# XJTU-Power-AI/charginghub-env

Measured on AMD Instinct MI355X. Metric: env-steps/sec at 65 536 parallel envs, higher is better.
Workload: dtype f64; 1 GPU; 65536 envs x hub [20 fast, 25 slow] (BASELINE.json configs[3]), fcev_permeate 0.01, random policy resident in HBM, reset every 96 steps, Philox streams; envs_per_gpu=65536, obs_dim=13, act_dim=47, work_order=XCD-aware (tiles, tail and level workgroups in contiguous eighths per XCD), graph=on, collective=none

## Files before the change

### charginghub-env_amd/csrc/chub_kernels.hip

```cpp
#include <hip/hip_runtime.h>
#include <hip/hip_ext.h>
#include <stdint.h>

#include "chub_device.h"
#include "chub_plan.h"

namespace chub {

typedef uint32_t u32x4 __attribute__((ext_vector_type(4)));
typedef uint32_t u32x2 __attribute__((ext_vector_type(2)));

__device__ __forceinline__ bool in_group(const StepArgs &sa, int64_t env) { return !sa.env_mask || sa.env_mask[env] != 0; }
__device__ __forceinline__ uint32_t env_clk(const StepArgs &sa, int64_t n_envs, int64_t env) {
    return sa.env_clk[(int64_t) (sa.tick & 1u) * n_envs + env];
}
__device__ __forceinline__ int64_t range_len(const StepArgs &sa) { return (int64_t) sa.env_hi - sa.env_lo + 1; }
__device__ __forceinline__ bool range_unit(const StepArgs &sa, int64_t i, int segments, int &seg, int64_t &env) {
    const int64_t R = range_len(sa);
    if (i >= (int64_t) segments * R) return false;
    seg = (i >= R ? 1 : 0) + (i >= 2 * R ? 1 : 0);
    env = sa.env_lo + (i - (int64_t) seg * R);
    return true;
}

// ... 1192 lines not shown
        float r_min, r_chg, r_max;
        if (MODE == MODE_COMPAT) {
            SumsF32 r = {0.0f, 0.0f, 0.0f};
            r.add(s_a, s_b, s_c, S);
            r_min = r.mn; r_chg = r.chg; r_max = r.mx;
        } else {
            SumsI64 r = {0, 0, 0};
            r.add(s_u, s_v, s_w, S);
            r_min = fixed64_to_kw(r.mn); r_chg = fixed64_to_kw(r.chg); r_max = fixed64_to_kw(r.mx);
        }
        rec_store(st.rec, sidx, r_min, r_chg, r_max, pkd_make(s_hdr[2], s_hdr[1], cars));
    }
}

template <bool RESET, int MODE>
__global__ __launch_bounds__(256) void k_slot_unit_any(const DevCtx *__restrict__ ctx, StepArgs sa, int k) {
    typedef float f32x2 __attribute__((ext_vector_type(2)));
    const HubParams &hp = ctx->hp;
    const SlotArrays &sl = ctx->sl;
    const StationArrays &st = ctx->st;
    const Tables &tb = ctx->tb;
    __shared__ float s_a[256], s_b[256], s_c[256];
    __shared__ uint32_t s_u[256], s_v[256], s_w[256];
    __shared__ float s_soc[256];
    __shared__ uint64_t s_ball[8];
    __shared__ int s_hdr[4];
    __shared__ int s_cnt;
    __shared__ float s_em[kMaxPiles], s_pw[kMaxPiles];
    __shared__ uint16_t s_cb[kMaxPiles], s_rk[kMaxPiles];
    const int tid = threadIdx.x, lane = tid & 63, wave = tid >> 6;
    const int env = (int) blockIdx.x;
    const int64_t N = hp.n_envs;
    if (!in_group(sa, env)) return;
    const int S = hp.S[k], chunks = (S + 255) >> 8;
    const bool fast = hp.type[k] == 0, cp = hp.constant_charging != 0;
    const int hub0 = k ? hp.S[0] : 0;
    const uint32_t idx0 = MODE == MODE_PHILOX ? (uint32_t) env * (uint32_t) (hp.S[0] + hp.S[1]) + (uint32_t) hub0
                                              : (uint32_t) hp.base[k] + (uint32_t) env * (uint32_t) S;
    const uint32_t sidx = (uint32_t) k * (uint32_t) N + (uint32_t) env;
    CHUB_G(const float) cls = tb.cls[k];
    if (tid == 0) s_cnt = 0;
    __syncthreads();

    float load = 0.0f;
    if (!RESET && sa.load_mode) {
        for (int slot = tid; slot < S; slot += 256) {
            const uint32_t idx = idx0 + (uint32_t) slot;
            float t_target = 0.0f, t_soc = 0.0f;
            int tl;
            if (MODE == MODE_COMPAT) {
                const u32x4 hot = ((CHUB_G(u32x4)) sl.hot)[idx];
                t_soc = __uint_as_float(hot.z);
                tl = hot_tl(hot.w);
                if (tl > 0) t_target = tb.ttab[k][hot_level(hot.w)];
            } else {
                const uint32_t w0 = sl.hot[idx];
                tl = ps_tl(w0);
                if (tl > 0) {
                    t_soc = (*(CHUB_G(const f32x2)) ((CHUB_G(const char)) cls + ((size_t) ps_cls(w0) * (kClsRow * 8u) + ps_n(w0) * 8u))).y;
                    t_target = tb.ttab[k][ps_lev(w0)];
                }
            }
            s_em[slot] = tl > 0 ? emergency_of(t_target, t_soc, tl) : 0.0f;
        }
        __syncthreads();
        for (int slot = tid; slot < S; slot += 256) {
            const uint32_t idx = idx0 + (uint32_t) slot;
            float power = 0.0f;
            bool car;
            if (MODE == MODE_COMPAT) {
                const u32x4 hot = ((CHUB_G(u32x4)) sl.hot)[idx];
                car = hot_tl(hot.w) != 0;
                power = __uint_as_float(hot.x);
            } else {
                const uint32_t w0 = sl.hot[idx];
                car = ps_tl(w0) > 0;
                if (car) power = (*(CHUB_G(const f32x2)) ((CHUB_G(const char)) cls + ((size_t) ps_cls(w0) * (kClsRow * 8u) + ps_n(w0) * 8u))).x;
            }
            const float em0 = s_em[slot];
            int rk = 0;
            for (int j = 0; j < S; j++) {
                const float ej = s_em[j];
                rk += (ej > em0 || (ej == em0 && j < slot)) ? 1 : 0;
            }
            s_rk[slot] = (uint16_t) rk;
            s_pw[rk] = car ? power : 0.0f;
            s_cb[rk] = car ? 1 : 0;
        }
        __syncthreads();
        load = catch_load(hp, sa, st, k, env, sidx);
        if (tid == 0) {
            float cum = 0.0f;
            int cars_before = 0;
            for (int q = 0; q < S; q++) {
                const int c = (int) s_cb[q];
                cum = __fadd_rn(cum, s_pw[q]);
                s_pw[q] = cum;
                s_cb[q] = (uint16_t) cars_before;
                cars_before += c;
            }
        }
        __syncthreads();
    }

    for (int c = 0; c < chunks; c++) {
        const int slot = (c << 8) + tid;
        const bool valid = slot < S;
        const uint32_t idx = idx0 + (uint32_t) slot;
        float a = 0.0f;
        if (!RESET && valid) a = sa.actions[(uint32_t) env * (uint32_t) hp.act_dim + (uint32_t) (hub0 + slot)];
        auto switched_on = [&](const float t_target, const float t_soc, const int tl) {
            if (!RESET && sa.load_mode) {
                const int rk = (int) s_rk[slot];
                return load_says_on(cp, fast, load, s_pw[rk], (int) s_cb[rk]);
            }
            return a >= kActOnThreshold || must_charge(t_target, t_soc, tl);
        };
        bool car;
        if constexpr (MODE == MODE_COMPAT) {
            CompatSlot s = {};
            float t_target = 0.0f;
            if (!RESET && valid) {
                const u32x4 hot = ((CHUB_G(u32x4)) sl.hot)[idx];
                s = CompatSlot::unpack(hot);
                if (s.tl > 0) t_target = tb.ttab[k][hot_level(hot.w)];
            }
            const bool on = s.tl > 0 && switched_on(t_target, s.t_soc, s.tl);
            if (on) car_step_compat(s, fast, cp, hp.cc);
            remove_car_compat(s, on);
            if (RESET) s.meta = 0;
            if (valid) ((CHUB_G(u32x4)) sl.hot)[idx] = s.pack();
            car = s.tl > 0;
        } else {
            PhiloxWord s = {};
            float t_target = 0.0f, t_soc = 0.0f;
            if (!RESET && valid) {
                s.w = sl.hot[idx];
                s.tl = ps_tl(s.w);
                if (s.tl > 0) {
                    t_soc = (*(CHUB_G(const f32x2)) ((CHUB_G(const char)) cls + ((size_t) ps_cls(s.w) * (kClsRow * 8u) + ps_n(s.w) * 8u))).y;
                    t_target = tb.ttab[k][ps_lev(s.w)];
                }
            }
            const bool on = s.tl > 0 && switched_on(t_target, t_soc, s.tl);
            car_step_word(s, on);
            if (RESET) s.w = 0u;
            if (valid) sl.hot[idx] = s.w;
            car = s.tl > 0;
        }
        const uint64_t be = __ballot(valid && !car);
        if (lane == 0 && be) atomicAdd(&s_cnt, __popcll(be));
    }
    __syncthreads();
    const int empties = s_cnt;

    CompatStream rs;
    if (tid == 0) {
        Received rc;
        if (MODE == MODE_COMPAT) {
            rs.load(ctx->cr, sa.rng_cur, env);
            rc = receive_car_streams<RESET>(rs, hp, sa, tb, k, env, fast, RESET ? 0 : pkd_line(st.rec[4u * sidx + 3u]), empties);
        } else {
            rc = receive_car_word<RESET>(st.pk[sa.tick & 1u][sidx], fast, empties);
        }
        s_hdr[0] = rc.assign; s_hdr[1] = rc.flow; s_hdr[2] = rc.line;
    }
    __syncthreads();
    const int assign = s_hdr[0];

    int base = 0, cars = 0;
    SumsF32 rf = {0.0f, 0.0f, 0.0f};
    SumsI64 ri = {0, 0, 0};
    for (int c = 0; c < chunks; c++) {
        const int slot = (c << 8) + tid;
        const bool valid = slot < S;
        const uint32_t idx = idx0 + (uint32_t) slot;
        float power = 0.0f, t_target = 0.0f, t_soc = 0.0f;
        int tl = 0;
        bool charge = false;
        if (valid) {
            if (MODE == MODE_COMPAT) {
                const u32x4 hot = ((CHUB_G(u32x4)) sl.hot)[idx];
                const CompatSlot cs = CompatSlot::unpack(hot);
                power = cs.power; t_soc = cs.t_soc; tl = cs.tl; charge = cs.charge;
                if (tl > 0) t_target = tb.ttab[k][hot_level(hot.w)];
            } else {
                const uint32_t w0 = sl.hot[idx];
                tl = ps_tl(w0);
                charge = (w0 & kPsChg) != 0u;
                if (tl > 0) {
                    const f32x2 row = *(CHUB_G(const f32x2)) ((CHUB_G(const char)) cls + ((size_t) ps_cls(w0) * (kClsRow * 8u) + ps_n(w0) * 8u));
                    power = row.x; t_soc = row.y;
                    t_target = tb.ttab[k][ps_lev(w0)];
                }
            }
        }
        bool car = tl > 0;
        const bool empty = valid && !car;
        const uint64_t be = __ballot(empty);
        if (lane == 0) s_ball[wave] = be;
        __syncthreads();
        int chunk_empties = 0, rank = base + prefix_count(be);
        for (int w = 0; w < 4; w++) {
            const int n = __popcll(s_ball[w]);
            chunk_empties += n;
            rank += w < wave ? n : 0;
        }
        if (MODE == MODE_COMPAT) {
            if (tid == 0) {
                int n_new = assign - base;
                n_new = n_new < 0 ? 0 : (n_new > chunk_empties ? chunk_empties : n_new);
                for (int rr = 0; rr < n_new; rr++) {
                    const CarDraw d = draw_car_streams(rs);
                    s_soc[rr] = d.soc;
                    s_v[rr] = (uint32_t) d.lev;
                    s_w[rr] = (uint32_t) d.late;
                }
            }
            __syncthreads();
        }
        if (empty && rank < assign) {
            if (MODE == MODE_COMPAT) {
                const int r = rank - base;
                const NewCar nc = add_car_compat(fast, s_soc[r], (int) s_v[r], (int) s_w[r], cp);
                t_target = nc.t_target; t_soc = nc.t_soc; tl = nc.stay; power = nc.power;
                ((CHUB_G(u32x4)) sl.hot)[idx] = compat_slot_of(nc).pack();
            } else {
                const PhiloxCar nc = add_car_philox(hp, sa, tb, k, env, hub0 + slot);
                t_target = nc.t_target; t_soc = nc.t_soc; tl = nc.stay; power = nc.power;
                sl.hot[idx] = nc.word;
                sl.stay8[idx] = (uint8_t) nc.stay;
            }
            car = tl > 0;
        }
        const bool urgent = car && must_charge(t_target, t_soc, tl);
        const uint64_t bc = __ballot(car);
        if (lane == 0) s_ball[4 + wave] = bc;
        if (MODE == MODE_COMPAT) {
            s_a[tid] = urgent ? power : 0.0f;
            s_b[tid] = charge ? power : 0.0f;
            s_c[tid] = car ? power : 0.0f;
        } else {
            const int q = kw_to_fixed(power);
            s_u[tid] = (uint32_t) (urgent ? q : 0);
            s_v[tid] = (uint32_t) (charge ? q : 0);
            s_w[tid] = (uint32_t) (car ? q : 0);
        }
        __syncthreads();
        cars += __popcll(s_ball[4]) + __popcll(s_ball[5]) + __popcll(s_ball[6]) + __popcll(s_ball[7]);
        if (tid == 0) {
            const int n = S - (c << 8) < 256 ? S - (c << 8) : 256;
            if (MODE == MODE_COMPAT) rf.add(s_a, s_b, s_c, n);
            else ri.add(s_u, s_v, s_w, n);
        }
        base += chunk_empties;
        __syncthreads();
    }
    if (tid == 0) {
        if (MODE == MODE_COMPAT) {
            rs.store(ctx->cr, sa.rng_cur, env);
            rec_store(st.rec, sidx, rf.mn, rf.chg, rf.mx, pkd_make(s_hdr[2], s_hdr[1], cars));
        } else {
            rec_store(st.rec, sidx, fixed64_to_kw(ri.mn), fixed64_to_kw(ri.chg), fixed64_to_kw(ri.mx), pkd_make(s_hdr[2], s_hdr[1], cars));
        }
    }
}

struct PackedArgs {
    uint32_t S[2], type[2];
    uint32_t n_envs, epb, magic, cls_delta;
    CHUB_G(uint32_t) state;
    CHUB_G(uint32_t) rec;
    CHUB_G(const uint32_t) pk;
    CHUB_G(const float) actions;
    CHUB_G(const float) cls0;
    CHUB_G(const float) ttab2;
    CHUB_G(const uint32_t) car_tape;
    uint32_t key[2], gid0, tick;
    const uint32_t *tick_base;
    uint32_t late[8];
    CHUB_G(const uint8_t) env_mask;
    uint32_t blk0;
    uint32_t xcd;
    CHUB_G(float) tail_act;
    CHUB_G(uint8_t) stay8;
};

typedef const uint32_t __attribute__((address_space(4))) *chub_sptr;
__device__ __forceinline__ uint32_t sload_u32(const void *p, int i) { return ((chub_sptr) (uintptr_t) p)[i]; }
__device__ __forceinline__ bool mask_is_empty(const StepArgs &sa) { return sa.skip_count != nullptr && sload_u32(sa.skip_count, 0) == 0u; }

#ifndef CHUB_ACT_NT
#define CHUB_ACT_NT 0
#endif
#if CHUB_ACT_NT
#define CHUB_ACT_LOAD(p) __builtin_nontemporal_load(p)
#else
#define CHUB_ACT_LOAD(p) (*(p))
#endif
#ifndef CHUB_ACC_COPIES
#define CHUB_ACC_COPIES 2
#endif
constexpr int kAccCopies = CHUB_ACC_COPIES;
#ifndef CHUB_EPI_ALL
#define CHUB_EPI_ALL 1
#endif
#define CHUB_AT(T_, base, byte_off) (*(CHUB_G(T_)) ((CHUB_G(char)) (base) + (uint32_t) (byte_off)))
template <int BLOCK, int T, bool RESET, bool BIG, bool MASKED, bool FUSED, bool BITS>
__device__ __forceinline__ void packed_records(const PackedArgs &pa, const uint32_t block_local, int *s_acc, const uint32_t *s_unit, u32x4 *s_rec) {
    const int lane = threadIdx.x & 63;
    const int S0 = (int) pa.S[0], S1 = (int) pa.S[1], St = S0 + S1;
    const int epb = (int) pa.epb, N = (int) pa.n_envs;
    const int env_first = (int) block_local * epb;
    const long long *s_acc64 = (const long long *) s_acc;
    __builtin_amdgcn_fence(__ATOMIC_RELEASE, "wavefront");
    __builtin_amdgcn_wave_barrier();
    __builtin_amdgcn_fence(__ATOMIC_ACQUIRE, "wavefront");
    for (int i = lane; i < 2 * epb; i += 64) {
        const int e = i >> 1, k = i & 1;
        const int env = env_first + e;
        if (env >= N) continue;
        if (MASKED && pa.env_mask[env] == 0) continue;
        const uint32_t su = (uint32_t) (k ? N : 0) + (uint32_t) env;
        if (!RESET && !FUSED && !BITS && k == 0) {
            typedef float f32x2_ __attribute__((ext_vector_type(2)));
            const uint32_t ai = ((uint32_t) env * (uint32_t) (St + 2) + (uint32_t) St) << 2;
            const f32x2_ tv = {CHUB_AT(const float, pa.actions, ai), CHUB_AT(const float, pa.actions, ai + 4u)};
            CHUB_AT(f32x2_, pa.tail_act, (uint32_t) env << 3) = tv;
        }
        uint32_t lf = s_unit[i];
        if ((k ? S1 : S0) == 0) {
            const uint32_t pk = CHUB_AT(const uint32_t, pa.pk, su << 2);
            const bool fast = (k ? pa.type[1] : pa.type[0]) == 0;
            int want, fl;
            if (RESET) {
                fl = fast ? (int) (int16_t) (pk & 0xFFFFu) : (int) ((pk >> 16) & 0xFFFFu);
                want = fl;
            } else {
                want = dk_want(pk);
                fl = dk_flow(pk);
            }
            const int as = want < 0 ? want : 0;
            int ln = want - as;
            ln = ln < kMaxLine ? ln : kMaxLine;
            lf = pkd_make(ln, fl, 0);
        }
        u32x4 rv;
        if (!BIG) {
            int a0 = 0, a1 = 0, a2 = 0, a3 = 0;
#pragma unroll
            for (int c = 0; c < kAccCopies; c++) {
                const int *acc = s_acc + 4 * i + c * 8 * epb;
                a0 += acc[0]; a1 += acc[1]; a2 += acc[2]; a3 += acc[3];
            }
            rv = u32x4{__float_as_uint(fixed_to_kw(a0)), __float_as_uint(fixed_to_kw(a1)), __float_as_uint(fixed_to_kw(a2)),
                       lf | ((uint32_t) a3 << 16)};
        } else {
            const long long *a64 = s_acc64 + 4 * i;
            rv = u32x4{__float_as_uint((float) a64[0] * (1.0f / 524288.0f)), __float_as_uint((float) a64[1] * (1.0f / 524288.0f)),
                       __float_as_uint((float) a64[2] * (1.0f / 524288.0f)), lf | ((uint32_t) a64[3] << 16)};
        }
        CHUB_AT(u32x4, pa.rec, su << 4) = rv;
        if (FUSED) s_rec[i] = rv;
    }
}
#undef CHUB_AT

struct NoHook {
    __device__ __forceinline__ void prefetch() {}
    __device__ __forceinline__ void park() {}
};
template <int BLOCK, int T, bool TAPE, bool RESET, bool BIG, bool MASKED, bool FUSED, typename Hook, bool BITS = false, bool PIPED = false>
__device__ __forceinline__ int slot_body_packed(const HubParams &hp, const StepArgs &sa, PackedArgs &pa, const Tables &tb,
                                                const uint32_t block_local, uint32_t *q_cnt, uint32_t *q_new,
                                                uint64_t *s_ball, int *s_acc, uint32_t *s_unit, Hook &hook, u32x4 *s_rec, uint32_t *s_uinfo) {
    typedef float f32x4 __attribute__((ext_vector_type(4)));
    typedef float f32x2 __attribute__((ext_vector_type(2)));
    constexpr int WAVES = BLOCK / 64;
    const int tid = threadIdx.x;
    const int lane = tid & 63, wave = tid >> 6;
    const int S0 = (int) pa.S[0], S1 = (int) pa.S[1], St = S0 + S1;
    const int epb = (int) pa.epb, N = (int) pa.n_envs;
    const int env_first = (int) block_local * epb;
    const uint32_t idx0 = (uint32_t) env_first * (uint32_t) St;
    CHUB_STAMP_DECL(16);
    CHUB_STAMP_REAL(12);
    CHUB_STAMP(0);
#define CHUB_AT(T_, base, byte_off) (*(CHUB_G(T_)) ((CHUB_G(char)) (base) + (uint32_t) (byte_off)))

    int e_[T], k_[T], slot[T];
    bool valid[T];
    uint32_t sidx[T];
    uint32_t s2[T];
    float act[T];
    u32x2 actw[T];
    int hs_[T];
    uint32_t pk_in[T];
#pragma unroll
    for (int j = 0; j < T; j++) {
        const int v = tid + j * BLOCK;
        e_[j] = (int) (__umul24((uint32_t) v, pa.magic) >> 20);
        const int hs = v - (int) __umul24((uint32_t) e_[j], (uint32_t) St);
        k_[j] = hs >= S0 ? 1 : 0;
        hs_[j] = hs;
        slot[j] = hs - (k_[j] ? S0 : 0);
        const int env = env_first + e_[j];
        valid[j] = e_[j] < epb && env < N;
        uint32_t served = 1u;
        if (MASKED && valid[j]) served = pa.env_mask[env];
        sidx[j] = (uint32_t) (k_[j] ? N : 0) + (uint32_t) env;
        asm volatile("" : "=v"(s2[j]), "=v"(act[j]), "=v"(pk_in[j]), "=v"(actw[j]));
        if (RESET) {
            s2[j] = 0u;
            act[j] = 0.0f;
        }
        if (valid[j]) {
            if (!RESET) {
                s2[j] = CHUB_AT(uint32_t, pa.state, (idx0 + (uint32_t) v) << 2);
                if (BITS) actw[j] = CHUB_AT(const u32x2, pa.actions, ((uint32_t) env * (((uint32_t) St + 63u) >> 6) + ((uint32_t) hs >> 6)) << 3);
                else act[j] = CHUB_ACT_LOAD((CHUB_G(const float)) ((CHUB_G(const char)) pa.actions + (uint32_t) ((idx0 + (uint32_t) v + 2u * (uint32_t) env) << 2)));
            }
            pk_in[j] = CHUB_AT(const uint32_t, pa.pk, sidx[j] << 2);
        }
        if (MASKED && valid[j]) valid[j] = served != 0u;
    }
    if (!TAPE) {
        pa.tick += sload_u32(pa.tick_base, 0);
        asm volatile("" : "+s"(pa.key[0]), "+s"(pa.key[1]), "+s"(pa.gid0), "+s"(pa.tick), "+s"(pa.late[0]), "+s"(pa.late[1]), "+s"(pa.late[2]),
                          "+s"(pa.late[3]), "+s"(pa.late[4]), "+s"(pa.late[5]), "+s"(pa.late[6]), "+s"(pa.late[7]));
    }
    CHUB_STAMP(1);
    if (FUSED) hook.prefetch();
    if (tid == 0) q_cnt[0] = 0;
    for (int i = tid; i < (BIG ? 16 : 8 * kAccCopies) * epb; i += BLOCK) s_acc[i] = 0;
    long long *s_acc64 = (long long *) s_acc;

    uint32_t w0[T];
    int tl[T];
    bool stays[T];
    f32x4 row[T];
    float ttg[T];
#pragma unroll
    for (int j = 0; j < T; j++) {
        asm volatile("" : "+v"(s2[j]));
        w0[j] = valid[j] ? s2[j] : 0u;
        tl[j] = ps_tl(w0[j]);
        stays[j] = tl[j] > 1;
        asm volatile("" : "=v"(row[j]), "=v"(ttg[j]));
        if (stays[j]) {
            row[j] = CHUB_AT(const f32x4, pa.cls0, (k_[j] ? pa.cls_delta : 0u) + (ps_cls(w0[j]) << 8) + (ps_n(w0[j]) << 3));
            ttg[j] = CHUB_AT(const float, pa.ttab2, (k_[j] ? 4096u : 0u) + (ps_lev(w0[j]) << 2));
        }
    }

    CHUB_STAMP(2);
    bool empty[T];
    uint64_t be[T];
#pragma unroll
    for (int j = 0; j < T; j++) {
        empty[j] = valid[j] && !stays[j];
        be[j] = __ballot(empty[j]);
        if (lane == 0) s_ball[wave + j * WAVES] = be[j];
    }
    if (FUSED) hook.park();
    CHUB_STAMP(3);
    __syncthreads();
    CHUB_STAMP(4);
    if (!BIG) {
        for (int u = tid; u < 2 * epb; u += BLOCK) {
            const int e = u >> 1, k = u & 1;
            const int Sk = k ? S1 : S0;
            const int U0 = e * St + (k ? S0 : 0), U1 = U0 + Sk;
            const int wv = U0 >> 6, lo = U0 & 63;
            const int hi0 = (U1 - (wv << 6)) < 64 ? (U1 - (wv << 6)) : 64;
            uint32_t info = (uint32_t) wv << 24;
            if (Sk > 0) {
                const uint64_t b0 = s_ball[wv];
                const uint64_t below_lo = lo ? (~0ull >> (64 - lo)) : 0ull, below_hi = ~0ull >> (64 - hi0);
                const int start_e = __popcll(b0 & below_lo), cnt0 = __popcll(b0 & below_hi & ~below_lo);
                const int over = U1 - ((wv + 1) << 6);
                const int cnt1 = over > 0 ? __popcll(s_ball[wv + 1] & (~0ull >> (64 - over))) : 0;
                info |= (uint32_t) start_e | ((uint32_t) cnt0 << 8) | ((uint32_t) (cnt0 + cnt1) << 16);
            }
            s_uinfo[u] = info;
        }
    }

    uint32_t w0n[T];
#pragma unroll
    for (int j = 0; j < T; j++) {
        if (BITS) asm volatile("" : "+v"(row[j]), "+v"(ttg[j]), "+v"(actw[j]));
        else asm volatile("" : "+v"(row[j]), "+v"(ttg[j]), "+v"(act[j]));
        const int u = 2 * e_[j] + k_[j];
        int *acc = s_acc + 4 * u + (BIG ? 0 : (lane & (kAccCopies - 1)) * 8 * epb);
        w0n[j] = 0u;
        if (stays[j]) {
            const float t_target = ttg[j];
            const bool bit_on = BITS && ((((hs_[j] & 32) ? actw[j].y : actw[j].x) >> (hs_[j] & 31)) & 1u) != 0u;
            const bool on = (BITS ? bit_on : act[j] >= kActOnThreshold) || must_charge(t_target, row[j].y, tl[j]);
            const float power = on ? row[j].z : row[j].x, t_soc = on ? row[j].w : row[j].y;
            const int q = kw_to_fixed(power);
            const bool urgent = must_charge(t_target, t_soc, tl[j] - 1);
            w0n[j] = (w0[j] & ~kPsChg) - 1u + (on ? (kPsStep | kPsChg) : 0u);
            if (!BIG) {
                atomicAdd((unsigned long long *) (acc + 2), (unsigned long long) (uint32_t) q | (1ull << 32));
                if (on || urgent)
                    atomicAdd((unsigned long long *) acc,
                              (unsigned long long) (urgent ? (uint32_t) q : 0u) | ((unsigned long long) (on ? (uint32_t) q : 0u) << 32));
            } else {
                unsigned long long *a64 = (unsigned long long *) (s_acc64 + 4 * u);
                atomicAdd(a64 + 2, (unsigned long long) q);
                atomicAdd(a64 + 3, 1ull);
                if (urgent) atomicAdd(a64 + 0, (unsigned long long) q);
                if (on) atomicAdd(a64 + 1, (unsigned long long) q);
            }
        }
    }
    CHUB_STAMP(5);
    if (!BIG) __syncthreads();
    CHUB_STAMP(6);

    int line[T], flow[T];
    bool adm[T];
    uint64_t ba[T];
    uint32_t n_push = 0;
#pragma unroll
    for (int j = 0; j < T; j++) {
        const int vw = wave + j * WAVES;
        int empties, rank;
        if (!BIG) {
            const uint32_t info = valid[j] ? s_uinfo[2 * e_[j] + k_[j]] : 0u;
            const int m = prefix_count(be[j]);
            empties = (int) ((info >> 16) & 255u);
            rank = (int) (info >> 24) == vw ? m - (int) (info & 255u) : m + (int) ((info >> 8) & 255u);
        } else {
            const int Sk = k_[j] ? S1 : S0;
            const int ub = e_[j] * St + (k_[j] ? S0 : 0) - vw * 64, ue = ub + Sk;
            empties = 0;
            rank = 0;
#pragma unroll
            for (int w = 0; w < WAVES * T; w++) {
                int lo = ub + (vw - w) * 64, hi = ue + (vw - w) * 64;
                lo = lo < 0 ? 0 : lo;
                hi = hi > 64 ? 64 : hi;
                if (hi > lo) {
                    const uint64_t m = (~0ull >> (64 - hi)) & (~0ull << lo);
                    const uint64_t b = (w == vw ? be[j] : s_ball[w]) & m;
                    empties += __popcll(b);
                    if (w < vw) rank += __popcll(b);
                    else if (w == vw) rank += prefix_count(b);
                }
            }
        }
        line[j] = 0;
        flow[j] = 0;
        int assign = 0;
        if (valid[j]) {
            const uint32_t pk = pk_in[j];
            int want;
            if (RESET) {
                const bool fast = (k_[j] ? pa.type[1] : pa.type[0]) == 0;
                flow[j] = fast ? (int) (int16_t) (pk & 0xFFFFu) : (int) ((pk >> 16) & 0xFFFFu);
                want = flow[j];
            } else {
                want = dk_want(pk);
                flow[j] = dk_flow(pk);
            }
            assign = want < empties ? want : empties;
            line[j] = want - assign;
            line[j] = line[j] < kMaxLine ? line[j] : kMaxLine;
        }
        adm[j] = empty[j] && rank < assign;
        ba[j] = __ballot(adm[j]);
        n_push += (uint32_t) __popcll(ba[j]);
    }
    if (n_push) {
        uint32_t base = 0;
        if (lane == 0) base = atomicAdd(&q_cnt[0], n_push);
        base = __shfl(base, 0);
#pragma unroll
        for (int j = 0; j < T; j++) {
            if (adm[j]) q_new[base + prefix_count(ba[j])] = (uint32_t) (tid + j * BLOCK);
            base += (uint32_t) __popcll(ba[j]);
        }
    }
#pragma unroll
    for (int j = 0; j < T; j++) {
        if (valid[j] && !adm[j]) CHUB_AT(uint32_t, pa.state, (idx0 + (uint32_t) (tid + j * BLOCK)) << 2) = w0n[j];
        if (valid[j] && slot[j] == 0) s_unit[2 * e_[j] + k_[j]] = pkd_make(line[j], flow[j], 0);
    }
    CHUB_STAMP(7);
    __syncthreads();
    CHUB_STAMP(8);
    constexpr bool ALL = RESET || CHUB_EPI_ALL || FUSED;
    if (!ALL && wave != WAVES - 1) return 0;
    if (PIPED && wave < WAVES / 2) return wave + 1;
    const uint32_t n_adm = q_cnt[0];
    for (uint32_t i = (uint32_t) (PIPED ? tid - (WAVES / 2) * 64 : (ALL ? tid : lane)); i < n_adm; i += (PIPED ? BLOCK - (WAVES / 2) * 64 : (ALL ? BLOCK : 64))) {
        const int src = (int) q_new[i];
        const int s_e = (int) (__umul24((uint32_t) src, pa.magic) >> 20);
        const int s_hs = src - (int) __umul24((uint32_t) s_e, (uint32_t) St);
        const int s_k = s_hs >= S0 ? 1 : 0;
        uint32_t c, lev;
        int late;
        if (TAPE) {
            const u32x2 tp = CHUB_AT(const u32x2, pa.car_tape, (idx0 + (uint32_t) src) << 3);
            c = tp.x;
            lev = tp.y & 0xFFFFu;
            late = (int) (tp.y >> 16);
        } else {
            PhiloxCtx p2{pa.key[0], pa.key[1], pa.tick, pa.gid0 + (uint32_t) (env_first + s_e)};
            const U4 o = p2.block(SITE_SOC, (uint32_t) s_hs, 0);
            c = o.v[0] >> kSocLevelShift;
            lev = o.v[1] % 1000u;
            late = 0;
#pragma unroll
            for (int j = 0; j < 8; j++) late += (o.v[2] >= pa.late[j]) ? 1 : 0;
            if (__any(o.v[2] >= pa.late[7])) {
#pragma unroll
                for (int j = 8; j < 16; j++) late += (o.v[2] >= tb.late_thr[j]) ? 1 : 0;
            }
        }
        f32x2 e0 = CHUB_AT(const f32x2, pa.cls0, (s_k ? pa.cls_delta : 0u) + (c << 8));
        float tt_ = CHUB_AT(const float, pa.ttab2, (s_k ? 4096u : 0u) + (lev << 2));
        asm volatile("" : "+v"(e0), "+v"(tt_));
        int st_ = (int) ceilf(__fsub_rn(tt_, e0.y)) + late;
        st_ = st_ > kMaxStay ? kMaxStay : st_;
        CHUB_AT(uint32_t, pa.state, (idx0 + (uint32_t) src) << 2) = st_ > 0 ? ps_make(st_, c, lev) : 0u;
        CHUB_AT(uint8_t, pa.stay8, idx0 + (uint32_t) src) = (uint8_t) st_;
        if (st_ > 0) {
            const int q = kw_to_fixed(e0.x);
            if (!BIG) {
                int *ac = s_acc + 4 * (2 * s_e + s_k) + (lane & (kAccCopies - 1)) * 8 * epb;
                atomicAdd((unsigned long long *) (ac + 2), (unsigned long long) (uint32_t) q | (1ull << 32));
                if (must_charge(tt_, e0.y, st_)) atomicAdd(ac, q);
            } else {
                unsigned long long *a64 = (unsigned long long *) (s_acc64 + 4 * (2 * s_e + s_k));
                atomicAdd(a64 + 2, (unsigned long long) q);
                atomicAdd(a64 + 3, 1ull);
                if (must_charge(tt_, e0.y, st_)) atomicAdd(a64 + 0, (unsigned long long) q);
            }
        }
    }
    CHUB_STAMP(9);
    if (FUSED) return wave == WAVES - 1 ? WAVES : wave + 1;
    if (ALL) {
        __syncthreads();
        CHUB_STAMP(10);
        CHUB_STAMP_REAL(13);
#if CHUB_TRACE
        if (sa.stamps_slot && tid == 0) {
            for (int i = 0; i <= 10; i++) sa.stamps_slot[(size_t) block_local * 16 + i] = stamp_[i];
            sa.stamps_slot[(size_t) block_local * 16 + 12] = stamp_[12];
            sa.stamps_slot[(size_t) block_local * 16 + 13] = stamp_[13];
        }
#endif
        if (wave != WAVES - 1) return 0;
    }
    packed_records<BLOCK, T, RESET, BIG, MASKED, false, BITS>(pa, block_local, s_acc, s_unit, nullptr);
#if CHUB_TRACE
    asm volatile("s_waitcnt vmcnt(0)" ::: "memory");
    CHUB_STAMP(11);
    if (sa.stamps_slot && lane == 0) sa.stamps_slot[(size_t) block_local * 16 + 11] = stamp_[11];
#endif
    return 0;
#undef CHUB_AT
}

template <int BLOCK, int T, bool TAPE, bool RESET, bool BIG, bool MASKED, bool BITS = false>
__global__ __launch_bounds__(BLOCK, (BLOCK <= 256 ? 8 : 2048 / BLOCK)) void k_slot_packed(const DevCtx *__restrict__ ctx, StepArgs sa, PackedArgs pa_in) {
    __shared__ uint32_t q_new[BLOCK * T];
    __shared__ uint32_t q_cnt[2];
    __shared__ uint64_t s_ball[BLOCK * T / 64 + 2];
    __shared__ __attribute__((aligned(16))) int s_acc[2 * BLOCK * T * kAccCopies];
    __shared__ uint32_t s_unit[BLOCK * T / 2];
    __shared__ uint32_t s_uinfo[BLOCK * T / 2];
    if (RESET && MASKED && mask_is_empty(sa)) return;
    PackedArgs pa = pa_in;
    asm volatile("" : "+s"(pa.S[0]), "+s"(pa.S[1]), "+s"(pa.type[0]), "+s"(pa.type[1]), "+s"(pa.n_envs), "+s"(pa.epb), "+s"(pa.magic),
                      "+s"(pa.cls_delta), "+s"(pa.state), "+s"(pa.rec), "+s"(pa.pk), "+s"(pa.actions), "+s"(pa.cls0), "+s"(pa.ttab2));
    NoHook hook;
    (void) slot_body_packed<BLOCK, T, TAPE, RESET, BIG, MASKED, false, NoHook, BITS>(ctx->hp, sa, pa, ctx->tb, xcd_order(blockIdx.x, pa.xcd, MASKED ? 0u : pa.xcd) + (MASKED ? pa.blk0 : 0u), q_cnt, q_new,
                                                                                     s_ball + 1, s_acc, s_unit, hook, nullptr, s_uinfo);
}

struct TailArgs {
    CHUB_G(const double) ou;
    CHUB_G(const double) price_noise;
    CHUB_G(const double) cap;
    CHUB_G(const int16_t) pv_day;
    CHUB_G(const int16_t) wd_day;
    CHUB_G(const uint8_t) q_len;
    CHUB_G(const uint8_t) hv_line;
    CHUB_G(const uint32_t) drw;
    CHUB_G(const uint8_t) drw_cnt;
    CHUB_G(uint32_t) rec;
    CHUB_G(const float) actions;
    uint32_t n_envs, act_dim, s_tot, xcd;
    CHUB_G(const float) tail_act;
    CHUB_G(const double) pv_row;
    CHUB_G(const double) wd_row;
    CHUB_G(const double) pv_row_now;
    CHUB_G(const double) wd_row_now;
    CHUB_G(const double) hy_table;
    const uint32_t *tick_base;
    double sin_t;
    uint32_t key[2], gid0, pad2;
};
inline TailArgs make_tail_args(const EnvArrays &ev, const StationArrays &st, const HubParams &hp, const StepArgs &sa, const PackedPtrs &pp,
                               bool reset) {
    TailArgs ta;
    const int t_next = reset ? 0 : (sa.t + 1) % 96;
    ta.tail_act = (hp.rng_mode == MODE_PHILOX && hp.packed && !sa.load_mode && !reset) ? (CHUB_G(const float)) st.tail_act : nullptr;
    if (sa.act_bits && !reset) ta.tail_act = (CHUB_G(const float)) sa.act_tail;
    ta.pv_row = (CHUB_G(const double)) (pp.tb->pvT + t_next * 100);
    ta.wd_row = (CHUB_G(const double)) (pp.tb->wdT + t_next * 150);
    ta.pv_row_now = (CHUB_G(const double)) (pp.tb->pvT + (reset ? 0 : sa.t) * 100);
    ta.wd_row_now = (CHUB_G(const double)) (pp.tb->wdT + (reset ? 0 : sa.t) * 150);
    ta.hy_table = (CHUB_G(const double)) pp.tb->hy_table;
    ta.tick_base = hp.tick_base;
    ta.sin_t = pp.sin96[t_next];
    ta.key[0] = hp.key[0];
    ta.key[1] = hp.key[1];
    ta.gid0 = (uint32_t) hp.env_id0;
    ta.pad2 = 0;
    ta.ou = (CHUB_G(const double)) ev.ou;
    ta.price_noise = (CHUB_G(const double)) ev.price_noise;
    ta.cap = (CHUB_G(const double)) ev.cap;
    ta.pv_day = (CHUB_G(const int16_t)) ev.pv_day;
    ta.wd_day = (CHUB_G(const int16_t)) ev.wd_day;
    ta.q_len = (CHUB_G(const uint8_t)) ev.q_len;
    ta.hv_line = (CHUB_G(const uint8_t)) ev.hv_line;
    ta.drw = (CHUB_G(const uint32_t)) ev.drw[sa.tick & 1u];
    ta.drw_cnt = (CHUB_G(const uint8_t)) ev.drw_cnt[sa.tick & 1u];
    ta.rec = (CHUB_G(uint32_t)) st.rec;
    ta.actions = (CHUB_G(const float)) sa.actions;
    ta.n_envs = (uint32_t) hp.n_envs;
    ta.act_dim = (uint32_t) hp.act_dim;
    ta.s_tot = (uint32_t) (hp.S[0] + hp.S[1]);
    ta.xcd = (hp.rng_mode == MODE_PHILOX && hp.packed && hp.xcd) ? 1u : 0u;
    return ta;
}

template <bool RESET, int MODE, int BLOCK>
__global__ __launch_bounds__(BLOCK, 7) void k_slot(const DevCtx *__restrict__ ctx, StepArgs sa, int64_t nb0) {
    const HubParams &hp = ctx->hp;
    __shared__ float lds_f[BLOCK];
    __shared__ uint32_t lds_u[2 * BLOCK];
    int k;
    int64_t bl;
    const int64_t bid = blockIdx.x;
    if (sa.station_filter >= 0) {
        k = sa.station_filter;
        bl = bid;
    } else {
        k = (bid >= nb0) ? 1 : 0;
        bl = k ? bid - nb0 : bid;
    }
    if (MODE == MODE_PHILOX) slot_body_wave<RESET, BLOCK>(hp, sa, ctx->sl, ctx->st, ctx->tb, k, bl, lds_f, lds_u);
    else if (hp.type[k] == 0) slot_body_compat<0, RESET, BLOCK>(hp, sa, ctx->sl, ctx->st, ctx->cr, ctx->tb, k, bl, lds_f, lds_u);
    else slot_body_compat<1, RESET, BLOCK>(hp, sa, ctx->sl, ctx->st, ctx->cr, ctx->tb, k, bl, lds_f, lds_u);
}

template <int TYPE, bool RESET, int BLOCK>
__device__ __forceinline__ void slot_body_curves(const HubParams &hp, const StepArgs &sa, const SlotArrays &sl, const StationArrays &st,
                                                 const Tables &tb, const int k, const int64_t block_local) {
    constexpr int WAVES = BLOCK / 64;
    typedef float f32x2 __attribute__((ext_vector_type(2)));
    const int tid = threadIdx.x;
    const int lane = tid & 63, wave = tid >> 6;
    const int H = hp.H[k], S = hp.S[k], logH = hp.logH[k];
    const int upw = 64 >> logH;
    const int uiw = lane >> logH;
    const int slot = lane & (H - 1);
    const int64_t N = hp.n_envs;
    const int env = (int) block_local * (WAVES * upw) + wave * upw + uiw;
    const bool unit_ok = env < (int) N && in_group(sa, env);
    const bool valid = unit_ok && slot < S;
    const uint64_t unit_mask = (H == 64) ? ~0ull : (((1ull << H) - 1ull) << (uiw << logH));
    const int hub_slot = (k ? hp.S[0] : 0) + slot;
    const uint32_t idx = (uint32_t) env * (uint32_t) (hp.S[0] + hp.S[1]) + (uint32_t) hub_slot;
    const uint32_t sidx = (uint32_t) k * (uint32_t) N + (uint32_t) env;
    const bool cp = hp.constant_charging != 0;

    uint32_t pk_in = 0, w0 = 0u;
    float a = 0.0f;
    f32x2 hv = {0.0f, 0.0f};
    if (unit_ok) pk_in = st.pk[sa.tick & 1u][sidx];
    if (!RESET && valid) {
        w0 = sl.wrd[idx];
        hv = *(CHUB_G(const f32x2)) ((CHUB_G(const float)) sl.hot + 2u * idx);
        a = sa.actions[(uint32_t) env * (uint32_t) hp.act_dim + (uint32_t) hub_slot];
    }
    int tl = ps_tl(w0);
    bool car = tl > 0;
    float power = hv.x, t_soc = hv.y;
    const float t_target = car ? tb.ttab[k][ps_lev(w0)] : 0.0f;
    const bool on = car && (a >= kActOnThreshold || must_charge(t_target, t_soc, tl));
    if (on && tl > 1) {
        float soc_new;
        car_step_curves<TYPE>(__fadd_rn(t_soc, 1.0f), cp, hp.cc, soc_new, power);
        t_soc = soc_to_time<TYPE>(soc_new, cp);
        w0 += kPsStep;
    }
    w0 &= ~kPsChg;
    if (car) {
        tl -= 1;
        w0 -= 1u;
        if (tl <= 0) {
            car = false;
            w0 = 0u;
            power = t_soc = 0.0f;
        }
    }
    const bool charge = on && car;
    if (charge) w0 |= kPsChg;

    const bool empty = valid && !car;
    const uint64_t be = __ballot(empty) & unit_mask;
    const int empties = __popcll(be);
    const int rank = prefix_count(be);
    Received rc = {0, 0, 0};
    if (unit_ok) rc = receive_car_word<RESET>(pk_in, TYPE == 0, empties);
    float tgt = t_target;
    if (empty && rank < rc.assign) {
        float soc;
        uint32_t lev;
        int late;
        if (sa.car_tape) {
            const uint32_t *tp = sa.car_tape + 2u * idx;
            soc = __uint_as_float(tp[0]);
            lev = tp[1] & 0xFFFFu;
            late = (int) (tp[1] >> 16);
        } else {
            const U4 o = car_block(hp, sa, env, hub_slot);
            soc = soc_from_word(tb.soc_d_icdf, o.v[0]);
            lev = o.v[1] % 1000u;
            late = late_from_word(tb.late_thr, o.v[2]);
        }
        tgt = tb.ttab[k][lev];
        t_soc = soc_to_time<TYPE>(soc, cp);
        power = time_to_power<TYPE>(t_soc, cp);
        int stay = (int) ceilf(__fsub_rn(tgt, t_soc)) + late;
        stay = stay > kMaxStay ? kMaxStay : stay;
        tl = stay;
        car = tl > 0;
        w0 = car ? ps_make(stay, 0u, lev) : 0u;
        sl.stay8[idx] = (uint8_t) stay;
        sl.soc0[idx] = soc;
    }

    const bool urgent = car && must_charge(tgt, t_soc, tl);
    const int q = kw_to_fixed(power);
    int i_min = urgent ? q : 0, i_max = car ? q : 0, i_chg = charge ? q : 0;
    unit_sums_dpp(H, i_min, i_max, i_chg);
    const int cars = __popcll(__ballot(car) & unit_mask);

    if (valid) {
        sl.wrd[idx] = w0;
        const f32x2 out = {car ? power : 0.0f, car ? t_soc : 0.0f};
        *(CHUB_G(f32x2)) ((CHUB_G(float)) sl.hot + 2u * idx) = out;
    }
    if (unit_ok && slot == 0) rec_store(st.rec, sidx, fixed_to_kw(i_min), fixed_to_kw(i_chg), fixed_to_kw(i_max), pkd_make(rc.line, rc.flow, cars));
}

template <bool RESET, int BLOCK>
__global__ __launch_bounds__(BLOCK) void k_slot_curves(const DevCtx *__restrict__ ctx, StepArgs sa, int64_t nb0) {
    const HubParams &hp = ctx->hp;
    const int64_t bid = blockIdx.x;
    const int k = (bid >= nb0) ? 1 : 0;
    const int64_t bl = k ? bid - nb0 : bid;
    if (hp.type[k] == 0) slot_body_curves<0, RESET, BLOCK>(hp, sa, ctx->sl, ctx->st, ctx->tb, k, bl);
    else slot_body_curves<1, RESET, BLOCK>(hp, sa, ctx->sl, ctx->st, ctx->tb, k, bl);
}

template <int BLOCK>
__global__ __launch_bounds__(BLOCK) void k_compat_empties(const DevCtx *__restrict__ ctx, StepArgs sa, int64_t nb0) {
    const HubParams &hp = ctx->hp;
    const int64_t bid = blockIdx.x;
    const int k = (bid >= nb0) ? 1 : 0;
    const int64_t bl = k ? bid - nb0 : bid;
    const int tid = threadIdx.x, lane = tid & 63, wave = tid >> 6;
    const int U = hp.U[k], S = hp.S[k];
    const int upw = 64 / U, uiw = lane / U, slot = lane - uiw * U;
    const int env = (int) bl * ((BLOCK / 64) * upw) + wave * upw + uiw;
    const bool unit_ok = uiw < upw && env < (int) hp.n_envs && in_group(sa, env);
    const bool valid = unit_ok && slot < S;
    const uint64_t unit_mask = (U == 64) ? ~0ull : (uiw < upw ? (((1ull << U) - 1ull) << (uiw * U)) : 0ull);
    uint32_t w = 0u;
    if (valid) w = ctx->sl.hot[4 * ((size_t) hp.base[k] + (size_t) env * (size_t) S + (size_t) slot) + 3];
    const bool empty = valid && (int) (w & 127u) <= 1;
    const uint64_t be = __ballot(empty) & unit_mask, be2 = __ballot(valid && (int) (w & 127u) <= 2) & unit_mask;
    if (unit_ok && slot == 0) {
        ctx->st.empt[(uint32_t) k * (uint32_t) hp.n_envs + (uint32_t) env] = (uint8_t) __popcll(be);
        ctx->st.empt2[(sa.tick + 1u) & 1u][(uint32_t) k * (uint32_t) hp.n_envs + (uint32_t) env] = (uint8_t) __popcll(be2);
    }
}

template <bool RESET, typename Stream, bool FORECOURT = false>
__device__ __forceinline__ void compat_walk_env(const DevCtx *__restrict__ ctx, const StepArgs &sa, const int env, Stream &rs) {
    const HubParams &hp = ctx->hp;
    const Tables &tb = ctx->tb;
    const StationArrays &st = ctx->st;
    const int64_t N = hp.n_envs;
    const uint32_t St = (uint32_t) (hp.S[0] + hp.S[1]);
    const uint32_t par = sa.tick & 1u;
    const bool far = !RESET && sa.walk_far != 0;
    const bool cp = hp.constant_charging != 0;
    for (int k = 0; k < 2; k++) {
        const int S = hp.S[k];
        const bool fast = hp.type[k] == 0;
        const uint32_t sidx = (uint32_t) k * (uint32_t) N + (uint32_t) env;
        int line = 0, empties = S;
        if (far) {
            const uint32_t wp = st.fa[par ^ 1u][sidx];
            line = (int) (wp >> 24);
            empties = (int) st.empt2[par][sidx] - (int) ((wp >> 16) & 255u) + (int) st.shrt[par ^ 1u][sidx];
        } else if (!RESET) {
            line = pkd_line(st.rec[4u * sidx + 3u]);
            empties = (int) st.empt[sidx];
        }
        const Received rc = receive_car_streams<RESET>(rs, hp, sa, tb, k, env, fast, line, empties);
        CHUB_G(u32x4) var = (CHUB_G(u32x4)) ctx->sl.var[par] + 2u * ((uint32_t) env * St + (uint32_t) (k ? hp.S[0] : 0));
        int n_short = 0;
        for (int rr = 0; rr < rc.assign; rr++) {
            const CarDraw d = draw_car_streams(rs);
            const NewCar nc = add_car_compat(fast, d.soc, d.lev, d.late, cp);
            var[2 * rr] = u32x4{__float_as_uint(nc.power), __float_as_uint(nc.t_target), __float_as_uint(nc.t_soc), (uint32_t) nc.stay | ((uint32_t) d.lev << 7)};
            var[2 * rr + 1] = u32x4{__float_as_uint(d.soc), 0u, 0u, 0u};
            n_short += (nc.stay <= 1) ? 1 : 0;
        }
        st.fa[par][sidx] = ((uint32_t) rc.flow & 0xFFFFu) | ((uint32_t) (rc.assign > 0 ? rc.assign : 0) << 16) | ((uint32_t) rc.line << 24);
        if (sa.walk_short) st.shrt[par][sidx] = (uint8_t) n_short;
    }
    if (FORECOURT && !RESET) {
        const int t_env = sa.env_clk ? clk_t(env_clk(sa, N, env)) : sa.t;
        CHUB_G(uint32_t) hv = ctx->ev.hv_pre[sa.tick & 1u] + (uint32_t) env * (uint32_t) hp.hv_w;
        const int arrive = (int) tb.cnt_hv[(uint32_t) t_env * (uint32_t) kLevels + (uint32_t) rs.level()];
        hv[0] = (uint32_t) arrive;
        for (int j = 0; j < arrive; j++) hv[1 + j] = __float_as_uint(arrive_soc_from(rs.normal_d(7.0, 3.0)));
    }
}

constexpr int kWalkCap = 256;
constexpr int kWalkStageWords = kWalkCap * 7 + 64;
struct WalkStage {
    double *yd, *r2d;
    float *yf, *r2f;
    uint32_t *meta;
    uint32_t *cnt;
};
__device__ __forceinline__ WalkStage walk_stage(uint32_t *base) {
    WalkStage g;
    g.yd = (double *) base;
    g.r2d = g.yd + kWalkCap;
    g.yf = (float *) (g.r2d + kWalkCap);
    g.r2f = g.yf + kWalkCap;
    g.meta = (uint32_t *) (g.r2f + kWalkCap);
    g.cnt = g.meta + kWalkCap;
    return g;
}
__device__ __forceinline__ void wave_sync_lds() {
// ... 2717 lines not shown
```

Baseline: 2.560 billion env-steps/s.

## Hand back admitted-slot state via LDS and prefetch record inputs early

Admitted slots no longer write state and stay8 to global memory from the scattered queue-processing lanes. They write the packed result into the LDS queue entry instead, and after the barrier the owning thread writes state for all its slots in coalesced order. By default this also defers the non-admitted state writes to that point. The last wave also prefetches tail actions and pk words for the records epilogue early, so those loads overlap the step body. An optional state-first load ordering is added behind a flag that is off by default. The cost is extra registers, an LDS round trip, and state writes that now sit after the barrier.

```diff
diff --git a/charginghub-env_amd/csrc/chub_kernels.hip b/charginghub-env_amd/csrc/chub_kernels.hip
--- a/charginghub-env_amd/csrc/chub_kernels.hip
+++ b/charginghub-env_amd/csrc/chub_kernels.hip
@@ -1518,12 +1518,22 @@
 #define CHUB_ACC_COPIES 2
 #endif
 constexpr int kAccCopies = CHUB_ACC_COPIES;
+#ifndef CHUB_HANDBACK
+#define CHUB_HANDBACK 2
+#endif
+#ifndef CHUB_HANDBACK_SMALL_TILE
+#define CHUB_HANDBACK_SMALL_TILE 0
+#endif
+#ifndef CHUB_STATE_FIRST
+#define CHUB_STATE_FIRST 0
+#endif
 #ifndef CHUB_EPI_ALL
 #define CHUB_EPI_ALL 1
 #endif
 #define CHUB_AT(T_, base, byte_off) (*(CHUB_G(T_)) ((CHUB_G(char)) (base) + (uint32_t) (byte_off)))
-template <int BLOCK, int T, bool RESET, bool BIG, bool MASKED, bool FUSED, bool BITS>
-__device__ __forceinline__ void packed_records(const PackedArgs &pa, const uint32_t block_local, int *s_acc, const uint32_t *s_unit, u32x4 *s_rec) {
+template <int BLOCK, int T, bool RESET, bool BIG, bool MASKED, bool FUSED, bool BITS, bool PRE = false>
+__device__ __forceinline__ void packed_records(const PackedArgs &pa, const uint32_t block_local, int *s_acc, const uint32_t *s_unit, u32x4 *s_rec,
+                                               const float pre_a0 = 0.0f, const float pre_a1 = 0.0f, const uint32_t pre_pk = 0u) {
     const int lane = threadIdx.x & 63;
     const int S0 = (int) pa.S[0], S1 = (int) pa.S[1], St = S0 + S1;
     const int epb = (int) pa.epb, N = (int) pa.n_envs;
@@ -1532,21 +1542,21 @@
     __builtin_amdgcn_fence(__ATOMIC_RELEASE, "wavefront");
     __builtin_amdgcn_wave_barrier();
     __builtin_amdgcn_fence(__ATOMIC_ACQUIRE, "wavefront");
-    for (int i = lane; i < 2 * epb; i += 64) {
+    auto record = [&](const int i, const bool pre) {
         const int e = i >> 1, k = i & 1;
         const int env = env_first + e;
-        if (env >= N) continue;
-        if (MASKED && pa.env_mask[env] == 0) continue;
+        if (env >= N) return;
+        if (MASKED && pa.env_mask[env] == 0) return;
         const uint32_t su = (uint32_t) (k ? N : 0) + (uint32_t) env;
         if (!RESET && !FUSED && !BITS && k == 0) {
             typedef float f32x2_ __attribute__((ext_vector_type(2)));
             const uint32_t ai = ((uint32_t) env * (uint32_t) (St + 2) + (uint32_t) St) << 2;
-            const f32x2_ tv = {CHUB_AT(const float, pa.actions, ai), CHUB_AT(const float, pa.actions, ai + 4u)};
+            const f32x2_ tv = {pre ? pre_a0 : CHUB_AT(const float, pa.actions, ai), pre ? pre_a1 : CHUB_AT(const float, pa.actions, ai + 4u)};
             CHUB_AT(f32x2_, pa.tail_act, (uint32_t) env << 3) = tv;
         }
         uint32_t lf = s_unit[i];
         if ((k ? S1 : S0) == 0) {
-            const uint32_t pk = CHUB_AT(const uint32_t, pa.pk, su << 2);
+            const uint32_t pk = pre ? pre_pk : CHUB_AT(const uint32_t, pa.pk, su << 2);
             const bool fast = (k ? pa.type[1] : pa.type[0]) == 0;
             int want, fl;
             if (RESET) {
@@ -1578,6 +1588,12 @@
         }
         CHUB_AT(u32x4, pa.rec, su << 4) = rv;
         if (FUSED) s_rec[i] = rv;
+    };
+    if (PRE) {
+        if (lane < 2 * epb) record(lane, true);
+        for (int i = lane + 64; i < 2 * epb; i += 64) record(i, false);
+    } else {
+        for (int i = lane; i < 2 * epb; i += 64) record(i, false);
     }
 }
 #undef CHUB_AT
@@ -1593,6 +1609,11 @@
     typedef float f32x4 __attribute__((ext_vector_type(4)));
     typedef float f32x2 __attribute__((ext_vector_type(2)));
     constexpr int WAVES = BLOCK / 64;
+    constexpr bool ALL = RESET || CHUB_EPI_ALL || FUSED;
+    constexpr bool LATE_TILE = BLOCK * T > 512 || CHUB_HANDBACK_SMALL_TILE;
+    constexpr bool HANDBACK = ALL && !FUSED && LATE_TILE && CHUB_HANDBACK != 0;
+    constexpr bool HB_LATE = HANDBACK && CHUB_HANDBACK == 2;
+    constexpr bool PRE = !FUSED && LATE_TILE;
     const int tid = threadIdx.x;
     const int lane = tid & 63, wave = tid >> 6;
     const int S0 = (int) pa.S[0], S1 = (int) pa.S[1], St = S0 + S1;
@@ -1630,7 +1651,7 @@
             s2[j] = 0u;
             act[j] = 0.0f;
         }
-        if (valid[j]) {
+        if (valid[j] && !(CHUB_STATE_FIRST && !RESET)) {
             if (!RESET) {
                 s2[j] = CHUB_AT(uint32_t, pa.state, (idx0 + (uint32_t) v) << 2);
                 if (BITS) actw[j] = CHUB_AT(const u32x2, pa.actions, ((uint32_t) env * (((uint32_t) St + 63u) >> 6) + ((uint32_t) hs >> 6)) << 3);
@@ -1639,6 +1660,35 @@
             pk_in[j] = CHUB_AT(const uint32_t, pa.pk, sidx[j] << 2);
         }
         if (MASKED && valid[j]) valid[j] = served != 0u;
+    }
+    if (CHUB_STATE_FIRST && !RESET) {
+        bool has[T];
+#pragma unroll
+        for (int j = 0; j < T; j++) {
+            has[j] = e_[j] < epb && env_first + e_[j] < N;
+            s2[j] = CHUB_AT(uint32_t, pa.state, (idx0 + (has[j] ? (uint32_t) (tid + j * BLOCK) : 0u)) << 2);
+        }
+#pragma unroll
+        for (int j = 0; j < T; j++) pk_in[j] = CHUB_AT(const uint32_t, pa.pk, (has[j] ? sidx[j] : (uint32_t) env_first) << 2);
+#pragma unroll
+        for (int j = 0; j < T; j++) {
+            const uint32_t env = (uint32_t) env_first + (has[j] ? (uint32_t) e_[j] : 0u);
+            const uint32_t v = has[j] ? (uint32_t) (tid + j * BLOCK) : 0u, hs = has[j] ? (uint32_t) hs_[j] : 0u;
+            if (BITS) actw[j] = CHUB_AT(const u32x2, pa.actions, (env * (((uint32_t) St + 63u) >> 6) + (hs >> 6)) << 3);
+            else act[j] = CHUB_ACT_LOAD((CHUB_G(const float)) ((CHUB_G(const char)) pa.actions + (uint32_t) ((idx0 + v + 2u * env) << 2)));
+        }
+    }
+    float rec_a0, rec_a1;
+    uint32_t rec_pk;
+    asm volatile("" : "=v"(rec_a0), "=v"(rec_a1), "=v"(rec_pk));
+    if (PRE && wave == WAVES - 1 && lane < 2 * epb && env_first + (lane >> 1) < N) {
+        const uint32_t env = (uint32_t) (env_first + (lane >> 1));
+        if (!RESET && !BITS && (lane & 1) == 0) {
+            const uint32_t ai = (env * (uint32_t) (St + 2) + (uint32_t) St) << 2;
+            rec_a0 = CHUB_AT(const float, pa.actions, ai);
+            rec_a1 = CHUB_AT(const float, pa.actions, ai + 4u);
+        }
+        if (((lane & 1) ? S1 : S0) == 0) rec_pk = CHUB_AT(const uint32_t, pa.pk, (((lane & 1) ? (uint32_t) N : 0u) + env) << 2);
     }
     if (!TAPE) {
         pa.tick += sload_u32(pa.tick_base, 0);
@@ -1740,8 +1790,10 @@
     bool adm[T];
     uint64_t ba[T];
     uint32_t n_push = 0;
+    uint32_t qpos[T];
 #pragma unroll
     for (int j = 0; j < T; j++) {
+        qpos[j] = 0u;
         const int vw = wave + j * WAVES;
         int empties, rank;
         if (!BIG) {
@@ -1796,19 +1848,21 @@
         base = __shfl(base, 0);
 #pragma unroll
         for (int j = 0; j < T; j++) {
-            if (adm[j]) q_new[base + prefix_count(ba[j])] = (uint32_t) (tid + j * BLOCK);
+            if (adm[j]) {
+                qpos[j] = base + (uint32_t) prefix_count(ba[j]);
+                q_new[qpos[j]] = (uint32_t) (tid + j * BLOCK);
+            }
             base += (uint32_t) __popcll(ba[j]);
         }
     }
 #pragma unroll
     for (int j = 0; j < T; j++) {
-        if (valid[j] && !adm[j]) CHUB_AT(uint32_t, pa.state, (idx0 + (uint32_t) (tid + j * BLOCK)) << 2) = w0n[j];
+        if (!HB_LATE && valid[j] && !adm[j]) CHUB_AT(uint32_t, pa.state, (idx0 + (uint32_t) (tid + j * BLOCK)) << 2) = w0n[j];
         if (valid[j] && slot[j] == 0) s_unit[2 * e_[j] + k_[j]] = pkd_make(line[j], flow[j], 0);
     }
     CHUB_STAMP(7);
     __syncthreads();
     CHUB_STAMP(8);
-    constexpr bool ALL = RESET || CHUB_EPI_ALL || FUSED;
     if (!ALL && wave != WAVES - 1) return 0;
     if (PIPED && wave < WAVES / 2) return wave + 1;
     const uint32_t n_adm = q_cnt[0];
@@ -1842,8 +1896,12 @@
         asm volatile("" : "+v"(e0), "+v"(tt_));
         int st_ = (int) ceilf(__fsub_rn(tt_, e0.y)) + late;
         st_ = st_ > kMaxStay ? kMaxStay : st_;
-        CHUB_AT(uint32_t, pa.state, (idx0 + (uint32_t) src) << 2) = st_ > 0 ? ps_make(st_, c, lev) : 0u;
-        CHUB_AT(uint8_t, pa.stay8, idx0 + (uint32_t) src) = (uint8_t) st_;
+        if (HANDBACK) {
+            q_new[i] = st_ > 0 ? ps_make(st_, c, lev) : (uint32_t) (uint8_t) st_ << 8;
+        } else {
+            CHUB_AT(uint32_t, pa.state, (idx0 + (uint32_t) src) << 2) = st_ > 0 ? ps_make(st_, c, lev) : 0u;
+            CHUB_AT(uint8_t, pa.stay8, idx0 + (uint32_t) src) = (uint8_t) st_;
+        }
         if (st_ > 0) {
             const int q = kw_to_fixed(e0.x);
             if (!BIG) {
@@ -1862,6 +1920,21 @@
     if (FUSED) return wave == WAVES - 1 ? WAVES : wave + 1;
     if (ALL) {
         __syncthreads();
+        if (HANDBACK) {
+#pragma unroll
+            for (int j = 0; j < T; j++) {
+                if (valid[j] && (HB_LATE || adm[j])) {
+                    uint32_t w = w0n[j];
+                    if (adm[j]) {
+                        const uint32_t hb = q_new[qpos[j]];
+                        const bool live = (hb & 31u) != 0u;
+                        w = live ? hb : 0u;
+                        CHUB_AT(uint8_t, pa.stay8, idx0 + (uint32_t) (tid + j * BLOCK)) = (uint8_t) (live ? (hb & 31u) : (hb >> 8));
+                    }
+                    CHUB_AT(uint32_t, pa.state, (idx0 + (uint32_t) (tid + j * BLOCK)) << 2) = w;
+                }
+            }
+        }
         CHUB_STAMP(10);
         CHUB_STAMP_REAL(13);
 #if CHUB_TRACE
@@ -1873,7 +1946,7 @@
 #endif
         if (wave != WAVES - 1) return 0;
     }
-    packed_records<BLOCK, T, RESET, BIG, MASKED, false, BITS>(pa, block_local, s_acc, s_unit, nullptr);
+    packed_records<BLOCK, T, RESET, BIG, MASKED, false, BITS, PRE>(pa, block_local, s_acc, s_unit, nullptr, rec_a0, rec_a1, rec_pk);
 #if CHUB_TRACE
     asm volatile("s_waitcnt vmcnt(0)" ::: "memory");
     CHUB_STAMP(11);
```

Result: no change. 2.561 billion env-steps/s, median of 4 (+0.0%).
